# agimus-project/agimus_controller

Hardware: AMD Instinct MI355X
Metric: MPC steps/sec (horizon=100, Panda 7-DoF) (higher is better)
Workload: dtype f64; 1 GPU; Panda 7-DoF sine_wave_configuration_space, ocp_goal_reaching.yaml costs, horizon=100, dt=0.01, batch=1024 independent MPC instances per GPU (seed 1234+b), closed loop on own prediction; horizon=100, batch_per_gpu=1024, global_batch=1024, max_iter=10

## Files before the change

agimus_controller_amd/backend.py:

```python

from __future__ import annotations

import ctypes as C
import os
import pathlib
import subprocess

import numpy as np

from . import _abi

_CSRC = pathlib.Path(__file__).resolve().parent / "csrc"
LIB_PATH = pathlib.Path(os.environ.get("AGX_LIB", _CSRC / "libagimus_hip.so"))
_LIB = None

EXPORTED_SYMBOLS = [
    "agx_last_error", "agx_device_count", "agx_row_nref", "agx_row_nr", "agx_ref_stride",
    "agx_model_create", "agx_model_destroy", "agx_ocp_create", "agx_ocp_destroy", "agx_ocp_set_stream",
    "agx_ocp_sync", "agx_ocp_set_refs", "agx_ocp_set_refs_device", "agx_ocp_solve", "agx_ocp_upload_x0",
    "agx_ocp_upload_warmstart", "agx_ocp_solve_resident", "agx_ocp_download", "agx_ocp_download_first", "agx_ocp_first_packed", "agx_ocp_set_geom_placement", "agx_ocp_reset_duals", "agx_traj_generic_create", "agx_traj_set_horizon_indexes", "agx_ocp_feedback_rollout", "agx_ocp_download_x0", "agx_model_frame_jacobian",
    "agx_ocp_shift_warmstart", "agx_ocp_x0_from_prediction", "agx_ocp_integrate", "agx_model_rnea",
    "agx_model_frame_placement", "agx_ocp_get_residuals", "agx_ocp_calc_diff", "agx_ocp_direction",
    "agx_ocp_time_kernel", "agx_ocp_profile", "agx_traj_sine_create", "agx_traj_set_window",
    "agx_traj_get_point", "agx_traj_warmstart_from_reference", "agx_ocp_mpc_step", "agx_ocp_qp_tiles", "agx_ocp_set_quorum",
    "agx_traj_cartesian_sine_create", "agx_ocp_set_refs_async", "agx_ocp_refs_activate", "agx_ocp_refs_wait", "agx_host_alloc", "agx_host_free",
    "agx_ocp_download_async", "agx_ocp_download_wait",
]


def _run(cmd, verbose):
    res = subprocess.run(cmd, capture_output=True, text=True)
    if verbose or res.returncode != 0:
        print(res.stdout, res.stderr)
    if res.returncode != 0:
        raise RuntimeError(f"{cmd[0]} failed ({res.returncode}): {res.stderr[-2000:]}")


def build(force: bool = False, verbose: bool = False) -> pathlib.Path:
    hdr = _CSRC.parent.parent / "include" / "agimus_hip.h"
    srcs = [_CSRC / "agimus_hip.hip"] + sorted(_CSRC.glob("*.hpp")) + [hdr, _CSRC / "agx_front.py"]
    if not force and LIB_PATH.exists() and LIB_PATH.stat().st_mtime >= max(s.stat().st_mtime for s in srcs):
        return LIB_PATH
    hipcc = os.environ.get("HIPCC", "/opt/rocm/bin/hipcc")
    base = [hipcc, "--offload-arch=gfx950", "-O3", "-std=c++17", "-fPIC"]
    if os.environ.get("AGX_BUILD_SPLIT", "1") == "0":
        _run(base + ["-shared", "-o", str(LIB_PATH), str(srcs[0])], verbose)
        return LIB_PATH
    import importlib.util

    spec = importlib.util.spec_from_file_location("agx_front", _CSRC / "agx_front.py")
    front = importlib.util.module_from_spec(spec)
    spec.loader.exec_module(front)
    obj = _CSRC.parent.parent / "build" / "obj"
    obj.mkdir(parents=True, exist_ok=True)
    names = [n for _, n, _ in front.prototypes(hdr.read_text())]
    procs = []
    for g in front.GROUPS:
        cmd = base + ["-c", f"-I{hdr.parent}"] + front.rename_flags(names, g) + ["-o", str(obj / f"agx_g{g}.o"), str(srcs[0])]
        procs.append((cmd, subprocess.Popen(cmd, stdout=subprocess.PIPE, stderr=subprocess.PIPE, text=True)))
    (obj / "agx_front.cpp").write_text(front.front_source(hdr.read_text()))
    _run(["g++", "-O2", "-std=c++17", "-fPIC", f"-I{hdr.parent}", "-c", "-o", str(obj / "agx_front.o"), str(obj / "agx_front.cpp")], verbose)
    failed = None
    for cmd, p in procs:
        out, err = p.communicate()
        if verbose or p.returncode != 0:
            print(out, err)
        if p.returncode != 0 and failed is None:
            failed = RuntimeError(f"hipcc failed ({p.returncode}) for {cmd[-1]} [{cmd[-3]}]: {err[-2000:]}")
    if failed:
        raise failed
    _run([hipcc, "--offload-arch=gfx950", "-shared", "-fPIC", "-o", str(LIB_PATH)] + [str(obj / f"agx_g{g}.o") for g in front.GROUPS]
         + [str(obj / "agx_front.o")], verbose)
    return LIB_PATH


def lib():
    global _LIB
    if _LIB is None:
        if not LIB_PATH.exists():
# ... 154 lines not shown
        _chk(lib().agx_ocp_upload_x0(self._h, _p(_f8(x0, (self.B, self.nx)))))

    def upload_warmstart(self, xs, us):
        xs = _f8(xs, (self.B, self.T + 1, self.nx))
        us = _f8(us, (self.B, self.T, self.nu))
        _chk(lib().agx_ocp_upload_warmstart(self._h, _p(xs), _p(us)))

    def solve_resident(self, max_iter, max_time=0.0):
        _chk(lib().agx_ocp_solve_resident(self._h, int(max_iter), C.c_double(max_time)))

    def download(self, want_K=True):
        xs = np.empty((self.B, self.T + 1, self.nx))
        us = np.empty((self.B, self.T, self.nu))
        K = np.empty((self.B, self.T, self.nu, self.nx)) if want_K else None
        st = np.zeros(self.B, dtype=_abi.STATUS_DTYPE)
        _chk(lib().agx_ocp_download(self._h, _p(xs), _p(us), _p(K), _p(st)))
        return xs, us, K, st

    def download_first(self, want_status=True, copy=True):
        ptr = C.POINTER(C.c_double)()
        stride = C.c_int(0)
        _chk(lib().agx_ocp_first_packed(self._h, C.byref(ptr), C.byref(stride)))
        addr = C.addressof(ptr.contents)
        cached = getattr(self, "_first_view", None)
        if cached is None or cached[0] != addr:
            cached = (addr, np.ctypeslib.as_array(ptr, shape=(self.B, stride.value)))
            self._first_view = cached
        buf = cached[1]
        nu, nx = self.nu, self.nx
        nk = nu * nx
        us0 = buf[:, :nu]
        K0 = buf[:, nu:nu + nk].reshape(self.B, nu, nx)
        x1 = buf[:, nu + nk:nu + nk + nx]
        if copy:
            us0, K0, x1 = us0.copy(), K0.copy(), x1.copy()
        st = None
        if want_status:
            q = buf[:, nu + nk + nx:]
            names = ("kkt", "cost", "merit", "gap_norm", "iter", "qp_iters", "solved", "flags")
            if copy:
                st = np.zeros(self.B, dtype=_abi.STATUS_DTYPE)
                for k, name in enumerate(names):
                    st[name] = q[:, k] if k < 4 else q[:, k].astype(np.int32)
            else:
                st = {name: q[:, k] for k, name in enumerate(names)}
        return us0, K0, x1, st

    def set_geom_placement(self, frame: int, se3_12):
        _chk(lib().agx_ocp_set_geom_placement(self._h, int(frame), _p(_f8(se3_12).reshape(12))))

    def set_quorum(self, sqp_fraction: float = 1.0, qp_fraction: float = 1.0):
        _chk(lib().agx_ocp_set_quorum(self._h, C.c_double(sqp_fraction), C.c_double(qp_fraction)))

    def reset_duals(self):
        _chk(lib().agx_ocp_reset_duals(self._h))

    def shift_warmstart(self):
        _chk(lib().agx_ocp_shift_warmstart(self._h))

    def x0_from_prediction(self):
        _chk(lib().agx_ocp_x0_from_prediction(self._h))

    def integrate(self, x, u):
        x = _f8(x).reshape(-1, self.nx)
        u = _f8(u).reshape(-1, self.nu)
        out = np.empty_like(x)
        _chk(lib().agx_ocp_integrate(self._h, x.shape[0], _p(x), _p(u), _p(out)))
        return out

    def rnea(self, q, v, a):
        q = _f8(q).reshape(-1, self.nv)
        v = _f8(v).reshape(-1, self.nv)
        a = _f8(a).reshape(-1, self.nv)
        tau = np.empty_like(q)
        _chk(lib().agx_model_rnea(self._h, q.shape[0], _p(q), _p(v), _p(a), _p(tau)))
        return tau

    def frame_placement(self, frame: int, q):
        q = _f8(q).reshape(-1, self.nv)
        out = np.empty((q.shape[0], 12))
        _chk(lib().agx_model_frame_placement(self._h, q.shape[0], int(frame), _p(q), _p(out)))
        return out

    def frame_jacobian(self, frame: int, q, local: bool = False):
        q = _f8(q).reshape(-1, self.nv)
        J = np.empty((q.shape[0], 6, self.nv))
        _chk(lib().agx_model_frame_jacobian(self._h, q.shape[0], int(frame), 1 if local else 0, _p(q), _p(J)))
        return J

    def residuals(self, row: int):
        nr = _abi.row_nr(self.po.running[row].kind, self.nv)
        out = np.empty((self.B, self.T, nr))
        _chk(lib().agx_ocp_get_residuals(self._h, int(row), _p(out)))
        return out

    def calc_diff(self, want_tiles=True):
        tiles = np.empty((self.B, self.T + 1, self.tile)) if want_tiles else None
        _chk(lib().agx_ocp_calc_diff(self._h, _p(tiles)))
        return tiles

    def qp_tiles(self):
        qs, as_ = C.c_int(0), C.c_int(0)
        _chk(lib().agx_ocp_qp_tiles(self._h, None, None, C.byref(qs), C.byref(as_)))
        qt = np.empty((self.B, self.T + 1, qs.value))
        aux = np.empty((self.B, self.T + 1, as_.value))
        _chk(lib().agx_ocp_qp_tiles(self._h, _p(qt), _p(aux), C.byref(qs), C.byref(as_)))
# ... 87 lines not shown
```

agimus_controller_amd/csrc/agimus_hip.hip:

```cpp

#include <hip/hip_runtime.h>

#include <algorithm>
#include <chrono>
#include <cmath>
#include <cstddef>
#include <cstdio>
#include <cstdlib>
#include <cstring>
#include <string>
#include <vector>

#include "agx_kernels.hpp"

namespace {

thread_local std::string g_err;
int fail(const std::string &msg) {
  g_err = msg;
  return -1;
}
#define HIPCHK(expr)                                                                                      \
  do {                                                                                                    \
    hipError_t e_ = (expr);                                                                               \
// ... 33 lines not shown
  int *d_shift_nodes = nullptr;
  bool general = false;
  double *d_auxg = nullptr;
  double *d_qt2 = nullptr, *d_cg = nullptr, *d_cjac = nullptr, *d_y = nullptr, *d_z = nullptr, *d_cx = nullptr, *d_admmstat = nullptr,
         *d_fac = nullptr,
         *d_segP = nullptr;
  bool admm_segments = true;
  int qt_size = 0, aux_size = 0;
  bool k1_lanes = true;
  bool lanes_ok = true;
  bool lanes_coll = false;
  bool speculate = true;
  bool gains_mfma = true;
  bool riccati_mx = true;
  int mx2_S = 0;
  double *d_mx2_elem = nullptr, *d_mx2_bnd = nullptr, *d_mx2_cl = nullptr;
  bool k1_fused = true;
  bool tile_carry = true;
  bool carry_static = false;
  bool carry_armed = false;
  int carry_k0 = 0;
  int head = 0;
  int n_carriable = -1;
  bool frames_uniform = true;
  double quorum_sqp = 1.0, quorum_qp = 1.0;
  bool con_lanes = true;
  bool con_wide = false;
  int con_cs = AGX_MAX_NC;
  bool admm_loop_always = false;
  bool admm_loop = true;
  int n_unfinished = 1 << 30;
  bool fold_publish = false;
  int n_cu = 256;
  bool no_empty = false;
  double *d_ref = nullptr;
  double *d_ref_back = nullptr;
  int *d_frames_back = nullptr;
  bool refs_pending = false, refs_pending_frames = false;
  hipStream_t copy_stream = nullptr;
  hipEvent_t ev_refs = nullptr, ev_snap = nullptr, ev_dl = nullptr;
  double *d_snap = nullptr;
  bool dl_pending = false;
  int *d_frames = nullptr;
  bool frames_set = false;
  DevState *d_state = nullptr;
  int *d_ndone = nullptr;
  unsigned long long *h_ndone = nullptr;
  unsigned long long *h_ndone_dev = nullptr;
  unsigned long long seq = 0;
  unsigned ls_handed = 0, ls_stale = 0;
  bool poll = true;
  double *d_first = nullptr, *h_first = nullptr;
  int first_stride = 0;
  double *d_scratch = nullptr;
  size_t scratch_bytes = 0;
  RefView rv{};
  double *d_traj = nullptr, *d_pts = nullptr;
  double *d_sine = nullptr;
  int n_points = 0;
  std::vector<int> hidx;
  int *d_hidx = nullptr;
  int win_k0 = 0;
  hipEvent_t ev0 = nullptr, ev1 = nullptr, ev_done = nullptr;
  int last_max_iter = 0;
  bool prof = false;
  std::vector<hipEvent_t> prof_ev;
  std::vector<int> prof_kind;
  double prof_ms[3] = {0, 0, 0};
  long long prof_n[3] = {0, 0, 0};
};

namespace {

int set_device(agx_ocp *o) {
  HIPCHK(hipSetDevice(o->device));
  return 0;
}

int pad_capacity(int nv);

void pad_rows(double *dst, const double *src, size_t rows, int blocks, int nvu, int nv, double fill) {
  for (size_t r = 0; r < rows; ++r)
    for (int b = 0; b < blocks; ++b) {
      double *d = dst + (r * blocks + b) * nv;
      const double *q = src + (r * blocks + b) * nvu;
      for (int i = 0; i < nvu; ++i) d[i] = q[i];
      for (int i = nvu; i < nv; ++i) d[i] = fill;
    }
}
void unpad_rows(double *dst, const double *src, size_t rows, int blocks, int nvu, int nv) {
  for (size_t r = 0; r < rows; ++r)
    for (int b = 0; b < blocks; ++b) {
      double *d = dst + (r * blocks + b) * nvu;
      const double *q = src + (r * blocks + b) * nv;
      for (int i = 0; i < nvu; ++i) d[i] = q[i];
    }
}
int up(agx_ocp *o, double *d_dst, const double *h_src, size_t rows, int blocks, double fill = 0.0) {
  if (!o->padded) {
    HIPCHK(hipMemcpyAsync(d_dst, h_src, sizeof(double) * rows * blocks * o->nv, hipMemcpyHostToDevice, o->stream));
    return 0;
  }
  o->stage.resize(rows * blocks * o->nv);
  pad_rows(o->stage.data(), h_src, rows, blocks, o->nvu, o->nv, fill);
  HIPCHK(hipMemcpyAsync(d_dst, o->stage.data(), sizeof(double) * o->stage.size(), hipMemcpyHostToDevice, o->stream));
  HIPCHK(hipStreamSynchronize(o->stream));
  return 0;
}
int down(agx_ocp *o, double *h_dst, const double *d_src, size_t rows, int blocks) {
  if (!o->padded) {
    HIPCHK(hipMemcpyAsync(h_dst, d_src, sizeof(double) * rows * blocks * o->nv, hipMemcpyDeviceToHost, o->stream));
    return 0;
  }
  o->stage.resize(rows * blocks * o->nv);
  HIPCHK(hipMemcpyAsync(o->stage.data(), d_src, sizeof(double) * o->stage.size(), hipMemcpyDeviceToHost, o->stream));
  HIPCHK(hipStreamSynchronize(o->stream));
  unpad_rows(h_dst, o->stage.data(), rows, blocks, o->nvu, o->nv);
  return 0;
}
int down_gains(agx_ocp *o, double *h_dst, const double *d_src, size_t n) {
  if (!o->padded) {
    HIPCHK(hipMemcpyAsync(h_dst, d_src, sizeof(double) * n * o->nu * o->nx, hipMemcpyDeviceToHost, o->stream));
    return 0;
  }
  const int nv = o->nv, nvu = o->nvu;
  o->stage.resize(n * nv * 2 * nv);
  HIPCHK(hipMemcpyAsync(o->stage.data(), d_src, sizeof(double) * o->stage.size(), hipMemcpyDeviceToHost, o->stream));
// ... 618 lines not shown
            if (n_conv < o->B && iter < max_qp) {
              hipLaunchKernelGGL(agx::k_admm_cap, dim3((o->B + 255) / 256), dim3(256), 0, o->stream, o->d_state, o->B, iter);
              HIPCHK(hipGetLastError());
            }
            break;
          }
        }
      }
      const long long units = (long long)o->B * o->T * 64;
      hipLaunchKernelGGL((agx::k_gains_to_u_big<NV>), dim3((int)((units + 255) / 256)), dim3(256), 0, o->stream, o->d_ocp, o->d_aux, o->d_Kws,
                         o->d_Kout, (const DevState *)nullptr);
      HIPCHK(hipGetLastError());
      return 0;
    } else {
      if constexpr (CH) if (o->con_wide) return admm_direction_nv7<NV, CH, true>(o, prefactor);
      return admm_direction_nv7<NV, CH, false>(o, prefactor);
    }
  });
}

int carry_invalidate(agx_ocp *o) {
  o->carry_armed = false;
  if (o->head != 0) {
    o->head = 0;
    HIPCHK(hipMemsetAsync((char *)o->d_ocp + offsetof(DevOcp, head), 0, sizeof(int), o->stream));
  }
  return 0;
}

int adopt_pending_refs(agx_ocp *o) {
  if (!o->refs_pending) return 0;
  if (carry_invalidate(o)) return -1;
  if (o->refs_pending_frames) o->frames_uniform = false;
  HIPCHK(hipStreamWaitEvent(o->stream, o->ev_refs, 0));
  std::swap(o->d_ref, o->d_ref_back);
  if (o->refs_pending_frames) std::swap(o->d_frames, o->d_frames_back);
  o->rv.base = o->d_ref;
  o->rv.bstride = (long long)(o->T + 1) * o->stride;
  o->rv.tstride = o->stride;
  o->rv.term_off = 0;
  o->rv.frames = o->refs_pending_frames ? o->d_frames : nullptr;
  o->refs_pending = false;
  return 0;
}
int ensure_copy_stream(agx_ocp *o) {
  if (o->copy_stream) return 0;
  HIPCHK(hipStreamCreateWithFlags(&o->copy_stream, hipStreamNonBlocking));
  HIPCHK(hipEventCreateWithFlags(&o->ev_refs, hipEventDisableTiming));
  HIPCHK(hipEventCreateWithFlags(&o->ev_snap, hipEventDisableTiming));
  HIPCHK(hipEventCreateWithFlags(&o->ev_dl, hipEventDisableTiming));
  return 0;
}

int line_search_rounds(agx_ocp *o, int it, int max_iter, bool *need_k1, int *n_done_out) {
  double *xs_t = o->d_xs + (size_t)o->B * (o->T + 1) * o->nx, *us_t = o->d_us + (size_t)o->B * o->T * o->nu;
  for (int round = 0; round < 10; ++round) {
    if (o->prof && round == 0 && it == 0) {
      if (prof_mark(o, 0, true)) return -1;
      if (launch_calc_qp(o, true, false, 1)) return -1;
      if (prof_mark(o, 0, false)) return -1;
      if (launch_calc_qp(o, false, true, 1)) return -1;
    } else if (launch_calc_qp(o, false, false, 1)) return -1;
    const unsigned long long seq = ++o->seq;
    int rc = dispatch(o->nv, o->chain, [&](auto NVc, auto CHc) -> int {
      constexpr int NV = decltype(NVc)::value;
      constexpr bool CH = decltype(CHc)::value;
      (void)CH;
      if constexpr (NV <= 7) if (o->has_con) {
        launch_con_eval<NV, CH>(o, xs_t, us_t, 1);
      }
      if constexpr (NV > 7) if (o->has_con) {
        const long long nodes = (long long)o->B * (o->T + 1);
        hipLaunchKernelGGL((agx::k_con_eval_wg<NV>), dim3((int)nodes), dim3(256), 0, o->stream, o->d_model, o->d_ocp, xs_t, us_t, o->d_cg, o->d_cjac,
                           o->d_nodestat, o->d_state, 1);
      }
      if (prof_mark(o, 2, true)) return -1;
      hipLaunchKernelGGL((agx::k_sqp_accept<NV>), dim3(o->B), dim3(128), 0, o->stream, o->d_ocp, o->d_xs, o->d_us, o->d_dx, o->d_du, xs_t, us_t,
                         o->d_qt, o->d_nodestat, o->d_state, it, max_iter, o->d_ndone, host_words(o, true, seq));
      HIPCHK(hipGetLastError());
      return prof_mark(o, 2, false);
    });
    if (rc) return rc;
    if (o->poll && o->fold_publish) {
      if (wait_stamp(o, 1, seq)) return -1;
    } else if (o->poll) {
      hipLaunchKernelGGL(agx::k_publish3, dim3(1), dim3(1), 0, o->stream, o->d_ndone, o->h_ndone_dev + 0, o->h_ndone_dev + 6, o->h_ndone_dev + 7,
                         o->h_ndone_dev + 8, o->h_ndone_dev + 1, seq);
      HIPCHK(hipGetLastError());
      if (wait_stamp(o, 1, seq)) return -1;
    } else {
      o->h_ndone[0] = 0; o->h_ndone[6] = 0; o->h_ndone[7] = 0; o->h_ndone[8] = 0;
      HIPCHK(hipMemcpyAsync(o->h_ndone + 8, o->d_ndone + 6, sizeof(int), hipMemcpyDeviceToHost, o->stream));
      HIPCHK(hipMemcpyAsync(o->h_ndone, o->d_ndone, sizeof(int), hipMemcpyDeviceToHost, o->stream));
      HIPCHK(hipMemcpyAsync(o->h_ndone + 6, o->d_ndone + 3, sizeof(int), hipMemcpyDeviceToHost, o->stream));
      HIPCHK(hipMemcpyAsync(o->h_ndone + 7, o->d_ndone + 4, sizeof(int), hipMemcpyDeviceToHost, o->stream));
      HIPCHK(hipStreamSynchronize(o->stream));
    }
    *n_done_out = (int)__atomic_load_n(o->h_ndone, __ATOMIC_ACQUIRE);
    const unsigned handed = (unsigned)__atomic_load_n(o->h_ndone + 6, __ATOMIC_ACQUIRE);
    const unsigned stale = (unsigned)__atomic_load_n(o->h_ndone + 7, __ATOMIC_ACQUIRE);
    o->n_carriable = (int)__atomic_load_n(o->h_ndone + 8, __ATOMIC_ACQUIRE);
    const bool more = handed != o->ls_handed;
    if (stale != o->ls_stale) *need_k1 = true;
    o->ls_handed = handed;
    o->ls_stale = stale;
    if (!more) break;
  }
  return 0;
}

int solve_resident(agx_ocp *o, int max_iter, double max_time, bool prologue_done = false, int carry_mode = 0) {
  if (max_iter <= 0) max_iter = 1000;
  o->last_max_iter = max_iter;
  o->n_carriable = -1;
  auto t0 = std::chrono::steady_clock::now();
  if (!prologue_done) {
    if (reset_state(o)) return -1;
    hipLaunchKernelGGL(agx::k_pin_x0, dim3((o->B * o->nx + 255) / 256), dim3(256), 0, o->stream, o->d_xs, o->d_x0, o->B, o->T, o->nx);
  }
  bool need_k1 = true;
  bool need_fixup = false;
  int prev_done = 0;
  for (int it = 0; it < max_iter; ++it) {
    const bool pair = o->speculate && it >= 1 && !o->has_con && o->nv <= 7;
    o->n_unfinished = o->B - prev_done;
    if (need_k1) {
      if (it == 0 && carry_mode != 0) {
        if (launch_calc_qp(o, false, false, 0, carry_mode == 2)) return -1;
      } else if (o->prof && it == 0) {
        if (prof_mark(o, 0, true)) return -1;
        if (launch_calc_qp(o, true, false)) return -1;
        if (prof_mark(o, 0, false)) return -1;
        if (launch_calc_qp(o, false, true)) return -1;
      } else if (launch_calc_qp(o, false, false)) return -1;
    }
    need_k1 = false;
    if (prof_mark(o, 1, true)) return -1;
    if (o->has_con && o->admm_prefactor && o->riccati_mx && o->nv <= 7 && !o->general) {
      if (admm_direction(o, true)) return -1;
    } else {
      if (launch_riccati(o, 1, pair, it)) return -1;
      if (o->has_con && admm_direction(o)) return -1;
    }
    if (prof_mark(o, 1, false)) return -1;
    const bool last = it + 1 == max_iter;
    if (prof_mark(o, 2, true)) return -1;
    const unsigned long long seq_head = ++o->seq;
    if (launch_step(o, it, max_iter, 1, !o->has_con, true, seq_head)) return -1;
    if (prof_mark(o, 2, false)) return -1;
    int n_done = 0;
    if (!pair && !o->has_con && (last || max_time > 0.0 || o->quorum_sqp < 1.0)) {
      if (launch_gains(o, 4)) return -1;
    }
    bool searching = true;
    if (o->poll && o->fold_publish && it >= 1) {
      if (wait_stamp(o, 1, seq_head)) return -1;
      n_done = (int)__atomic_load_n(o->h_ndone, __ATOMIC_ACQUIRE);
      o->n_carriable = (int)__atomic_load_n(o->h_ndone + 8, __ATOMIC_ACQUIRE);
      searching = n_done < o->B;
    } else if (o->prof || o->no_empty) {
      if (read_int(o, o->d_ndone, 0, 1, &n_done)) return -1;
      searching = n_done < o->B;
      if (!searching && read_int(o, o->d_ndone + 6, 8, 1, &o->n_carriable)) return -1;
    }
    if (searching && line_search_rounds(o, it, max_iter, &need_k1, &n_done)) return -1;
    if (last) { need_fixup = need_fixup || !pair; break; }
    if (!pair && n_done > prev_done) need_fixup = true;
    prev_done = n_done;
    if (n_done >= quorum_count(o->B, o->quorum_sqp)) {
      if (n_done < o->B) o->last_max_iter = it + 1;
      break;
    }
    if (max_time > 0.0) {
      const double el = std::chrono::duration<double>(std::chrono::steady_clock::now() - t0).count();
      if (el > max_time) { need_fixup = need_fixup || !pair; o->last_max_iter = it + 1; break; }
    }
  }
  if (!o->has_con && need_fixup && launch_gains(o, 2)) return -1;
  return prof_collect(o);
}

}

extern "C" {

const char *agx_last_error(void) { return g_err.c_str(); }

int agx_device_count(void) {
  int n = 0;
  if (hipGetDeviceCount(&n) != hipSuccess) return 0;
  return n;
}

int agx_row_nref(int kind, int nv) {
  switch (kind) {
    case AGX_RES_STATE: return 2 * nv;
    case AGX_RES_CONTROL: return nv;
    case AGX_RES_CONTROL_GRAV: return 0;
    case AGX_RES_FRAME_PLACEMENT: return 12;
    case AGX_RES_FRAME_TRANSLATION: return 3;
    case AGX_RES_FRAME_ROTATION: return 9;
    case AGX_RES_FRAME_VELOCITY: return 6;
    case AGX_RES_COLLISION: return 0;
  }
  return -1;
}
int agx_row_nr(int kind, int nv) {
  switch (kind) {
    case AGX_RES_STATE: return 2 * nv;
    case AGX_RES_CONTROL: return nv;
    case AGX_RES_CONTROL_GRAV: return nv;
    case AGX_RES_FRAME_PLACEMENT: return 6;
    case AGX_RES_FRAME_TRANSLATION: return 3;
    case AGX_RES_FRAME_ROTATION: return 3;
    case AGX_RES_FRAME_VELOCITY: return 6;
    case AGX_RES_COLLISION: return 1;
  }
  return -1;
// ... 60 lines not shown
  return 0;
}
void agx_model_destroy(agx_model *m) { delete m; }

int agx_ocp_create(const agx_model *m, const agx_ocp_desc *d, int batch, int device, agx_ocp **out) {
  if (!m || !d || !out) return fail("agx_ocp_create: null argument");
  if (batch < 1) return fail("agx_ocp_create: batch must be positive");
  if (d->horizon < 1) return fail("agx_ocp_create: horizon must be positive");
  if (d->n_running_rows > AGX_MAX_ROWS || d->n_terminal_rows > AGX_MAX_ROWS) return fail("agx_ocp_create: too many cost rows");
  int ndev = 0;
  if (hipGetDeviceCount(&ndev) != hipSuccess || ndev <= 0) return fail("agx_ocp_create: no HIP device available (this library has no CPU path)");
  if (device < 0 || device >= ndev) return fail("agx_ocp_create: bad device index");
  for (int r = 0; r < d->n_running_rows + d->n_terminal_rows; ++r) {
    const agx_cost_row &row = r < d->n_running_rows ? d->running_rows[r] : d->terminal_rows[r - d->n_running_rows];
    switch (row.kind) {
      case AGX_RES_STATE: case AGX_RES_CONTROL: case AGX_RES_FRAME_PLACEMENT: case AGX_RES_FRAME_TRANSLATION: case AGX_RES_FRAME_ROTATION:
      case AGX_RES_COLLISION: break;
      case AGX_RES_CONTROL_GRAV: case AGX_RES_FRAME_VELOCITY:
        if (m->h.nv > 7) return fail("agx_ocp_create: ControlGrav / FrameVelocity rows are implemented for nv <= 7");
        if (row.kind == AGX_RES_FRAME_VELOCITY && (row.frame < 0 || row.frame >= m->h.nframes || row.frame_b < 0 || row.frame_b > 2))
          return fail("agx_ocp_create: FrameVelocity row needs a valid frame and a reference frame 0 (WORLD), 1 (LOCAL) or 2 (LOCAL_WORLD_ALIGNED)");
        break;
      default: return fail("agx_ocp_create: residual kind " + std::to_string(row.kind) + " is not implemented on the HIP path yet");
    }
    if (row.activation != AGX_ACT_WEIGHTED_QUAD && (row.kind == AGX_RES_CONTROL_GRAV || row.kind == AGX_RES_FRAME_VELOCITY))
      return fail("agx_ocp_create: ActivationModelExp / QuadExp are not implemented for ControlGrav / FrameVelocity residuals");
    if (row.activation != AGX_ACT_WEIGHTED_QUAD && !(row.alpha > 0.0)) return fail("agx_ocp_create: activation alpha must be positive");
    if ((row.kind == AGX_RES_FRAME_PLACEMENT || row.kind == AGX_RES_FRAME_TRANSLATION || row.kind == AGX_RES_FRAME_ROTATION) &&
        (row.frame < 0 || row.frame >= m->h.nframes))
      return fail("agx_ocp_create: frame id out of range");
    if (row.kind == AGX_RES_COLLISION) {
      if (row.frame < 0 || row.frame >= m->h.nframes || row.frame_b < 0 || row.frame_b >= m->h.nframes)
        return fail("agx_ocp_create: collision pair refers to a geometry frame out of range");
      if (!agx::frame_has_geometry(m->h, row.frame) || !agx::frame_has_geometry(m->h, row.frame_b))
        return fail("agx_ocp_create: collision pair refers to a frame without geometry (radius 0, no box)");
      if (agx::frame_is_box(m->h, row.frame) && agx::frame_is_box(m->h, row.frame_b))
        return fail("agx_ocp_create: box / box collision pairs are not supported");
    }
  }
  agx_ocp *o = new agx_ocp();
  o->hm = m->h;
  o->nv = m->h.nv; o->nx = 2 * o->nv; o->nu = o->nv;
  o->chain = m->h.is_chain != 0;
  if (const char *e = getenv("AGX_K1_LANES")) o->k1_lanes = (e[0] != '0');
  if (const char *e = getenv("AGX_SPECULATE_GAINS")) o->speculate = (e[0] != '0');
  if (const char *e = getenv("AGX_GAINS_MFMA")) o->gains_mfma = (e[0] != '0');
  if (const char *e = getenv("AGX_RICCATI_MX")) o->riccati_mx = (e[0] != '0');
  if (const char *e = getenv("AGX_NO_EMPTY_LAUNCHES")) o->no_empty = (e[0] != '0');
  o->fold_publish = batch <= 204;
  if (const char *e = getenv("AGX_FOLD_PUBLISH")) o->fold_publish = (e[0] != '0');
  if (const char *e = getenv("AGX_ADMM_LOOP")) { o->admm_loop = (e[0] != '0'); o->admm_loop_always = (e[0] == '2'); }
  if (const char *e = getenv("AGX_K1_FUSED")) o->k1_fused = (e[0] != '0');
  if (const char *e = getenv("AGX_TILE_CARRY")) o->tile_carry = (e[0] != '0');
  o->T = d->horizon; o->B = batch; o->device = device;
  {
    int n = 0;
    if (hipDeviceGetAttribute(&n, hipDeviceAttributeMultiprocessorCount, device) == hipSuccess && n > 0) o->n_cu = n;
  }
  o->tile = AGX_TILE_DOUBLES(o->nv);
  const int ld = o->nv <= 8 ? 8 : 32;
  o->qt_size = 6 * o->nv * ld + 5 * ld + 8;
  o->aux_size = 4 * o->nv * ld + 3 * ld;
  o->stride = agx_ref_stride(d, o->nv);
  o->dt.assign(d->dt, d->dt + d->horizon);
  std::memset(&o->ho, 0, sizeof(o->ho));
  o->ho.T = o->T; o->ho.B = o->B; o->ho.stride = o->stride;
  fill_rows(d->running_rows, d->n_running_rows, o->nv, m->nvu, o->ho.rows[0]);
  fill_rows(d->terminal_rows, d->n_terminal_rows, o->nv, m->nvu, o->ho.rows[1]);
  o->ho.tol = d->termination_tolerance;
  o->ho.mu_dyn = d->mu_dynamic;
  o->ho.mu_con = d->mu_constraint;
  o->nvu = m->nvu;
  o->padded = o->nvu != o->nv;
  o->stride_u = agx_ref_stride(d, o->nvu);
  if (o->padded) {
    for (int lay = 0; lay < 2; ++lay) {
      const DevRows &R = o->ho.rows[lay];
      o->refmap[lay].assign(o->stride, -1);
      o->reffill[lay].assign(o->stride, 0.0);
      int off_u = 0;
      for (int r = 0; r < R.n; ++r) {
        const int kind = R.kind[r], nref_u = agx_row_nref(kind, o->nvu), nr_u = agx_row_nr(kind, o->nvu);
        o->refmap[lay][R.off[r]] = off_u;
        for (int k = 0; k < R.nref[r]; ++k) {
          const int ku = user_component(kind, k, o->nv, o->nvu, true);
          o->refmap[lay][R.off[r] + 1 + k] = ku >= 0 ? off_u + 1 + ku : -1;
        }
        for (int k = 0; k < R.nr[r]; ++k) {
          const int ku = user_component(kind, k, o->nv, o->nvu, false);
          o->refmap[lay][R.off[r] + 1 + R.nref[r] + k] = ku >= 0 ? off_u + 1 + nref_u + ku : -1;
          if (ku < 0) o->reffill[lay][R.off[r] + 1 + R.nref[r] + k] = 1.0;
        }
        off_u += 1 + nref_u + nr_u;
      }
    }
  }
  {
    const int wc_r = wide_class(d->running_constraints, d->n_running_constraints, false),
              wc_t = wide_class(d->terminal_constraints, d->n_terminal_constraints, true);
    const bool wide_model = o->nv <= 7 && o->chain, wide_ok = wide_model && wc_r == 0 && wc_t == 0;
    bool wide = false;
    if (const char *e = getenv("AGX_CON_WIDE")) wide = wide_ok && e[0] == '1';
    if (!wide && (fill_cons(d->running_constraints, d->n_running_constraints, o->nv, o->nvu, m->h, o->ho.cons[0], false) ||
                  fill_cons(d->terminal_constraints, d->n_terminal_constraints, o->nv, o->nvu, m->h, o->ho.cons[1], true))) {
      if (wide_model && (wc_r == 2 || wc_t == 2)) {
        delete o;
// ... 156 lines not shown
  (void)hipEventCreate(&o->ev1);
  (void)hipEventCreateWithFlags(&o->ev_done, hipEventDisableTiming);
  o->rv.base = o->d_ref;
  o->rv.bstride = (long long)(T + 1) * o->stride;
  o->rv.tstride = o->stride;
  o->rv.term_off = 0;
  o->rv.frames = nullptr;
  if (reset_state(o) || hipStreamSynchronize(o->stream) != hipSuccess) { agx_ocp_destroy(o); return fail("agx_ocp_create: state reset failed"); }
  *out = o;
  return 0;
}

void agx_ocp_destroy(agx_ocp *o) {
  if (!o) return;
  (void)hipSetDevice(o->device);
  if (o->stream) (void)hipStreamSynchronize(o->stream);
  if (o->copy_stream) (void)hipStreamSynchronize(o->copy_stream);
  void *ptrs[] = {o->d_mx2_elem, o->d_mx2_bnd, o->d_mx2_cl, o->d_ref_back, o->d_frames_back, o->d_snap, o->d_model, o->d_ocp, o->d_dt, o->d_xs, o->d_us, o->d_x0, o->d_tiles, o->d_Kws, o->d_kws, o->d_Kout, o->d_dx,
                  o->d_du, o->d_ref, o->d_frames, o->d_state, o->d_ndone, o->d_scratch, o->d_traj, o->d_pts, o->d_sine, o->d_qt, o->d_aux, o->d_w, o->d_nodestat,
                  o->d_qt2, o->d_cg, o->d_cjac, o->d_y, o->d_z, o->d_cx, o->d_admmstat, o->d_fac, o->d_hidx, o->d_auxg, o->d_shift_nodes, o->d_segP, o->d_Kws_lqr, o->d_kws_lqr};
  for (void *p : ptrs)
    if (p) (void)hipFree(p);
  if (o->h_ndone) (void)hipHostFree(o->h_ndone);
  if (o->ev0) (void)hipEventDestroy(o->ev0);
  if (o->ev1) (void)hipEventDestroy(o->ev1);
  if (o->ev_done) (void)hipEventDestroy(o->ev_done);
  if (o->ev_refs) (void)hipEventDestroy(o->ev_refs);
  if (o->ev_snap) (void)hipEventDestroy(o->ev_snap);
  if (o->ev_dl) (void)hipEventDestroy(o->ev_dl);
  if (o->copy_stream) (void)hipStreamDestroy(o->copy_stream);
  if (o->d_first && !o->poll) (void)hipFree(o->d_first);
  if (o->h_first) (void)hipHostFree(o->h_first);
  if (o->own_stream && o->stream) (void)hipStreamDestroy(o->stream);
  delete o;
}

int agx_ocp_set_stream(agx_ocp *o, void *hip_stream) {
  if (!o) return fail("null handle");
  if (set_device(o)) return -1;
  if (o->stream) HIPCHK(hipStreamSynchronize(o->stream));
  if (hip_stream) {
    if (o->own_stream && o->stream) (void)hipStreamDestroy(o->stream);
    o->stream = (hipStream_t)hip_stream;
    o->own_stream = false;
  } else if (!o->own_stream) {
    HIPCHK(hipStreamCreateWithFlags(&o->stream, hipStreamNonBlocking));
    o->own_stream = true;
  }
  return 0;
}

int agx_ocp_sync(agx_ocp *o) {
  if (!o) return fail("null handle");
  if (set_device(o)) return -1;
  HIPCHK(hipStreamSynchronize(o->stream));
  return 0;
}

int agx_ocp_set_quorum(agx_ocp *o, double sqp_fraction, double qp_fraction) {
  if (!o) return fail("null handle");
  if (!(sqp_fraction > 0.0 && sqp_fraction <= 1.0) || !(qp_fraction > 0.0 && qp_fraction <= 1.0))
    return fail("agx_ocp_set_quorum: fractions must be in (0, 1]");
  o->quorum_sqp = sqp_fraction;
  o->quorum_qp = qp_fraction;
  return 0;
}

int agx_ocp_reset_duals(agx_ocp *o) {
  if (!o) return fail("null handle");
  if (set_device(o)) return -1;
  if (o->has_con) HIPCHK(hipMemsetAsync(o->d_y, 0, sizeof(double) * (size_t)o->B * (o->T + 1) * o->con_cs, o->stream));
  hipLaunchKernelGGL(agx::k_reset_rho, dim3((o->B + 255) / 256), dim3(256), 0, o->stream, o->d_state, o->B);
  HIPCHK(hipGetLastError());
  HIPCHK(hipStreamSynchronize(o->stream));
  return 0;
}

int agx_ocp_set_geom_placement(agx_ocp *o, int frame, const double *se3) {
  if (!o || !se3) return fail("agx_ocp_set_geom_placement: null argument");
  if (frame < 0 || frame >= o->hm.nframes) return fail("agx_ocp_set_geom_placement: frame out of range");
  if (set_device(o)) return -1;
  if (carry_invalidate(o)) return -1;
  std::memcpy(o->hm.frame_placement[frame], se3, sizeof(double) * 12);
  HIPCHK(hipMemcpyAsync((char *)o->d_model + offsetof(DevModel, frame_placement) + sizeof(double) * 12 * frame, o->hm.frame_placement[frame],
                        sizeof(double) * 12, hipMemcpyHostToDevice, o->stream));
  HIPCHK(hipStreamSynchronize(o->stream));
  return 0;
}

int agx_ocp_set_refs(agx_ocp *o, const double *ref_tile, const int32_t *frame_ids) {
  if (!o || !ref_tile) return fail("agx_ocp_set_refs: null argument");
  if (set_device(o)) return -1;
  if (carry_invalidate(o)) return -1;
  if (frame_ids) o->frames_uniform = false;
  if (o->refs_pending) { HIPCHK(hipEventSynchronize(o->ev_refs)); o->refs_pending = false; }
  const size_t n = (size_t)o->B * (o->T + 1);
  if (o->padded) {
    o->stage.resize(n * o->stride);
    pad_ref_tile(o, o->stage.data(), ref_tile, o->B, o->T);
    ref_tile = o->stage.data();
  }
  HIPCHK(hipMemcpyAsync(o->d_ref, ref_tile, sizeof(double) * n * o->stride, hipMemcpyHostToDevice, o->stream));
  if (frame_ids) HIPCHK(hipMemcpyAsync(o->d_frames, frame_ids, sizeof(int) * n * AGX_MAX_ROWS, hipMemcpyHostToDevice, o->stream));
  HIPCHK(hipStreamSynchronize(o->stream));
  o->rv.base = o->d_ref;
  o->rv.bstride = (long long)(o->T + 1) * o->stride;
  o->rv.tstride = o->stride;
  o->rv.term_off = 0;
// ... 115 lines not shown
  return 0;
}

int agx_ocp_upload_x0(agx_ocp *o, const double *x0) {
  if (!o || !x0) return fail("agx_ocp_upload_x0: null argument");
  if (set_device(o)) return -1;
  if (up(o, o->d_x0, x0, o->B, 2)) return -1;
  HIPCHK(hipStreamSynchronize(o->stream));
  return 0;
}

int agx_ocp_upload_warmstart(agx_ocp *o, const double *xs_ws, const double *us_ws) {
  if (!o || !xs_ws || !us_ws) return fail("agx_ocp_upload_warmstart: null argument");
  if (set_device(o)) return -1;
  if (carry_invalidate(o)) return -1;
  if (up(o, o->d_xs, xs_ws, (size_t)o->B * (o->T + 1), 2)) return -1;
  if (up(o, o->d_us, us_ws, (size_t)o->B * o->T, 1)) return -1;
  HIPCHK(hipStreamSynchronize(o->stream));
  return 0;
}

int agx_ocp_solve_resident(agx_ocp *o, int max_iter, double max_time) {
  if (!o) return fail("null handle");
  if (set_device(o)) return -1;
  if (carry_invalidate(o)) return -1;
  return solve_resident(o, max_iter, max_time);
}

int agx_ocp_download(agx_ocp *o, double *xs, double *us, double *K, agx_status *st) {
  if (!o) return fail("null handle");
  if (set_device(o)) return -1;
  const size_t B = o->B, T = o->T, nx = o->nx, nu = o->nu;
  (void)nx; (void)nu;
  if (xs && down(o, xs, o->d_xs, B * (T + 1), 2)) return -1;
  if (us && down(o, us, o->d_us, B * T, 1)) return -1;
  if (K && down_gains(o, K, o->d_Kout, B * T)) return -1;
  std::vector<DevState> hs;
  if (st) {
    hs.resize(B);
    HIPCHK(hipMemcpyAsync(hs.data(), o->d_state, sizeof(DevState) * B, hipMemcpyDeviceToHost, o->stream));
  }
  HIPCHK(hipStreamSynchronize(o->stream));
  if (st)
    for (size_t b = 0; b < B; ++b) {
      st[b].kkt = hs[b].kkt; st[b].cost = hs[b].cost; st[b].merit = hs[b].merit; st[b].gap_norm = hs[b].gap;
      st[b].iter = hs[b].done ? hs[b].iter : o->last_max_iter;
      st[b].qp_iters = hs[b].qp_iters; st[b].solved = hs[b].solved; st[b].flags = hs[b].flags;
    }
  return 0;
}

int agx_ocp_first_packed(agx_ocp *o, const double **host, int *stride) {
  if (!o || !host) return fail("agx_ocp_first_packed: null argument");
  if (set_device(o)) return -1;
  const int FS = o->nu + o->nu * o->nx + o->nx + 8;
  if (!o->h_first) {
    if (o->poll && hipHostMalloc((void **)&o->h_first, sizeof(double) * (size_t)o->B * FS, hipHostMallocMapped | hipHostMallocCoherent) != hipSuccess) {
      (void)hipGetLastError();
      o->poll = false;
    }
    if (!o->poll) HIPCHK(hipHostMalloc((void **)&o->h_first, sizeof(double) * (size_t)o->B * FS, hipHostMallocDefault));
    if (o->poll) {
      HIPCHK(hipHostGetDevicePointer((void **)&o->d_first, o->h_first, 0));
    } else {
      HIPCHK(hipMalloc((void **)&o->d_first, sizeof(double) * (size_t)o->B * FS));
    }
    o->first_stride = FS;
  }
  const long long n = (long long)o->B * FS;
  hipLaunchKernelGGL(agx::k_pack_first, dim3((int)((n + 255) / 256)), dim3(256), 0, o->stream, o->d_us, o->d_Kout, o->d_xs, o->d_state,
                     o->d_first, o->B, o->T, o->nx, o->nu, o->last_max_iter);
  HIPCHK(hipGetLastError());
  if (o->poll) {
    const unsigned long long seq = ++o->seq;
    if (publish(o, 3, 2, o->d_ndone, seq)) return -1;
    if (wait_stamp(o, 2, seq)) return -1;
  } else {
    HIPCHK(hipMemcpyAsync(o->h_first, o->d_first, sizeof(double) * n, hipMemcpyDeviceToHost, o->stream));
    HIPCHK(hipStreamSynchronize(o->stream));
  }
  if (o->padded) {
    const int nv = o->nv, nvu = o->nvu, FSu = nvu + nvu * 2 * nvu + 2 * nvu + 8;
    o->h_first_u.resize((size_t)o->B * FSu);
    for (int b = 0; b < o->B; ++b) {
      const double *r = o->h_first + (size_t)b * FS;
      double *w = o->h_first_u.data() + (size_t)b * FSu;
      unpad_rows(w, r, 1, 1, nvu, nv);
      for (int i = 0; i < nvu; ++i) unpad_rows(w + nvu + (size_t)i * 2 * nvu, r + nv + (size_t)i * 2 * nv, 1, 2, nvu, nv);
      unpad_rows(w + nvu + nvu * 2 * nvu, r + nv + nv * 2 * nv, 1, 2, nvu, nv);
      std::memcpy(w + nvu + nvu * 2 * nvu + 2 * nvu, r + nv + nv * 2 * nv + 2 * nv, sizeof(double) * 8);
    }
    *host = o->h_first_u.data();
    if (stride) *stride = FSu;
    return 0;
  }
  *host = o->h_first;
  if (stride) *stride = FS;
  return 0;
}

int agx_ocp_download_first(agx_ocp *o, double *us0, double *K0, double *x1, agx_status *st) {
  const double *h = nullptr;
  int FS = 0;
  if (agx_ocp_first_packed(o, &h, &FS)) return -1;
  const int nu = o->nvu, nx = 2 * o->nvu, nk = nu * nx;
  for (int b = 0; b < o->B; ++b) {
    const double *r = h + (size_t)b * FS;
    if (us0) std::memcpy(us0 + (size_t)b * nu, r, sizeof(double) * nu);
    if (K0) std::memcpy(K0 + (size_t)b * nk, r + nu, sizeof(double) * nk);
    if (x1) std::memcpy(x1 + (size_t)b * nx, r + nu + nk, sizeof(double) * nx);
    if (st) {
      const double *q = r + nu + nk + nx;
      st[b].kkt = q[0]; st[b].cost = q[1]; st[b].merit = q[2]; st[b].gap_norm = q[3];
      st[b].iter = (int)q[4]; st[b].qp_iters = (int)q[5]; st[b].solved = (int)q[6]; st[b].flags = (int)q[7];
    }
  }
  return 0;
}

int agx_ocp_solve(agx_ocp *o, const double *x0, const double *xs_ws, const double *us_ws, int max_iter, double max_time,
                  double *xs, double *us, double *K, agx_status *st) {
  if (!o || !x0 || !xs_ws || !us_ws) return fail("agx_ocp_solve: null argument");
  if (agx_ocp_upload_x0(o, x0)) return -1;
  if (agx_ocp_upload_warmstart(o, xs_ws, us_ws)) return -1;
  if (solve_resident(o, max_iter, max_time)) return -1;
  return agx_ocp_download(o, xs, us, K, st);
}

int agx_ocp_shift_warmstart(agx_ocp *o) {
  if (!o) return fail("null handle");
// ... 525 lines not shown
  if (n_substeps < 1 || !(dt_sub > 0.0)) return fail("agx_ocp_feedback_rollout: bad sub-stepping");
  if (set_device(o)) return -1;
  double *d_dist = nullptr;
  if (disturbance) {
    if (ensure_scratch(o, sizeof(double) * o->B * o->nu)) return -1;
    d_dist = o->d_scratch;
    if (up(o, d_dist, disturbance, o->B, 1)) return -1;
  }
  return dispatch(o->nv, o->chain, [&](auto NVc, auto CHc) -> int {
    constexpr int NV = decltype(NVc)::value;
    constexpr bool CH = decltype(CHc)::value;
    hipLaunchKernelGGL((agx::k_feedback_rollout<NV, CH>), dim3((o->B + 63) / 64), dim3(64), 0, o->stream, o->d_model, o->d_us, o->d_Kout, o->d_x0,
                       d_dist, o->B, o->T, n_substeps, dt_sub);
    HIPCHK(hipGetLastError());
    if (disturbance) HIPCHK(hipStreamSynchronize(o->stream));
    return 0;
  });
}

int agx_ocp_mpc_step(agx_ocp *o, int k0, int max_iter, int first) {
  if (!o) return fail("null handle");
  if (set_device(o)) return -1;
  if (agx_traj_set_window(o, k0)) return -1;
  bool prologue_done = false;
  const size_t lds = sizeof(double) * (size_t)o->T * (o->nx + o->nu);
  const bool one_launch = o->nv <= 8 && lds <= 60 * 1024;
  const bool carry = o->carry_static && o->carry_armed && first != 1 && k0 == o->carry_k0 + 1 && one_launch && o->hidx.empty() && o->frames_uniform;
  const int carry_mode = !carry ? 0 : (o->n_carriable == o->B ? 2 : 1);
  if (!carry && carry_invalidate(o)) return -1;
  o->carry_armed = false;
  if (first == 1) {
    if (ws_from_ref(o, k0, 1)) return -1;
  } else {
    if (one_launch) {
      if (carry) o->head = (o->head + 1) % o->T;
      int rc = dispatch(o->nv, o->chain, [&](auto NVc, auto CHc) -> int {
        constexpr int NV = decltype(NVc)::value;
        constexpr bool CH = decltype(CHc)::value;
        if constexpr (NV <= 8) {
          hipLaunchKernelGGL((agx::k_mpc_prologue<NV, CH>), dim3(o->B), dim3(128), lds, o->stream, o->d_model, o->d_ocp, o->d_dt, o->d_xs,
                             o->d_us, o->d_x0, o->d_state, o->d_ndone, first == 0 ? 1 : 0, carry ? 1 : 0, o->head,
                             (int *)((char *)o->d_ocp + offsetof(DevOcp, head)));
          HIPCHK(hipGetLastError());
        }
        return 0;
      });
      if (rc) return rc;
      prologue_done = true;
    } else {
      if (first == 0 && agx_ocp_x0_from_prediction(o)) return -1;
      if (agx_ocp_shift_warmstart(o)) return -1;
    }
  }
  if (solve_resident(o, max_iter, 0.0, prologue_done, carry_mode)) return -1;
  o->carry_armed = o->carry_static;
  o->carry_k0 = k0;
  return 0;
}

}
```

include/agimus_hip.h:

```cpp
#ifndef AGIMUS_HIP_H
#define AGIMUS_HIP_H

#include <stddef.h>
#include <stdint.h>

#ifdef __cplusplus
extern "C" {
#endif

#define AGX_MAX_ROWS 8
#define AGX_MAX_NV 32

enum agx_residual_kind {
  AGX_RES_STATE = 0,
  AGX_RES_CONTROL = 1,
  AGX_RES_CONTROL_GRAV = 2,
  AGX_RES_FRAME_PLACEMENT = 3,
  AGX_RES_FRAME_TRANSLATION = 4,
  AGX_RES_FRAME_ROTATION = 5,
  AGX_RES_FRAME_VELOCITY = 6,
  AGX_RES_COLLISION = 7
};

enum agx_activation_kind {
// ... 42 lines not shown
  const double *frame_box;
} agx_model_desc;

typedef struct agx_ocp_desc {
  int32_t horizon;
  const double *dt;
  int32_t n_running_rows;
  const agx_cost_row *running_rows;
  int32_t n_terminal_rows;
  const agx_cost_row *terminal_rows;
  double termination_tolerance;
  int32_t max_qp_iters;
  double eps_abs, eps_rel;
  double mu_dynamic, mu_constraint;
  int32_t use_filter_line_search;
  int32_t n_running_constraints;
  const agx_constraint_row *running_constraints;
  int32_t n_terminal_constraints;
  const agx_constraint_row *terminal_constraints;
} agx_ocp_desc;

typedef struct agx_status {
  double kkt;
  double cost;
  double merit;
  double gap_norm;
  int32_t iter;
  int32_t qp_iters;
  int32_t solved;
  int32_t flags;
} agx_status;

#define AGX_TILE_DOUBLES(nv) (4 * (nv) * (nv) + 2 * (nv) * (nv) + 2 * (nv) + 2 * (nv) + (nv) + 4 * (nv) * (nv) + 2 * (nv) * (nv) + (nv) * (nv) + 1)

typedef struct agx_model agx_model;
typedef struct agx_ocp agx_ocp;

const char *agx_last_error(void);
int agx_device_count(void);

int agx_row_nref(int kind, int nv);
int agx_row_nr(int kind, int nv);
int agx_ref_stride(const agx_ocp_desc *desc, int nv);

int agx_model_create(const agx_model_desc *desc, agx_model **out);
void agx_model_destroy(agx_model *m);

int agx_ocp_create(const agx_model *m, const agx_ocp_desc *desc, int batch, int device, agx_ocp **out);
void agx_ocp_destroy(agx_ocp *ocp);
int agx_ocp_set_stream(agx_ocp *ocp, void *hip_stream);
int agx_ocp_sync(agx_ocp *ocp);
int agx_ocp_set_geom_placement(agx_ocp *ocp, int frame, const double *se3);
int agx_ocp_set_quorum(agx_ocp *ocp, double sqp_fraction, double qp_fraction);
int agx_ocp_reset_duals(agx_ocp *ocp);

int agx_ocp_set_refs(agx_ocp *ocp, const double *ref_tile, const int32_t *frame_ids);
int agx_ocp_set_refs_async(agx_ocp *ocp, const double *ref_tile, const int32_t *frame_ids);
int agx_ocp_refs_activate(agx_ocp *ocp);
int agx_ocp_refs_wait(agx_ocp *ocp);
int agx_host_alloc(size_t bytes, void **out);
int agx_host_free(void *p);
int agx_ocp_set_refs_device(agx_ocp *ocp, const double *d_ref_tile, const int32_t *d_frame_ids, int adopt);

int agx_ocp_solve(agx_ocp *ocp, const double *x0, const double *xs_ws, const double *us_ws,
                  int max_iter, double max_time, double *xs, double *us, double *K, agx_status *st);

int agx_ocp_upload_x0(agx_ocp *ocp, const double *x0);
int agx_ocp_upload_warmstart(agx_ocp *ocp, const double *xs_ws, const double *us_ws);
int agx_ocp_solve_resident(agx_ocp *ocp, int max_iter, double max_time);
int agx_ocp_download(agx_ocp *ocp, double *xs, double *us, double *K, agx_status *st);
int agx_ocp_download_async(agx_ocp *ocp, double *xs, double *us, double *K);
int agx_ocp_download_wait(agx_ocp *ocp);
int agx_ocp_download_first(agx_ocp *ocp, double *us0, double *K0, double *x1, agx_status *st);
int agx_ocp_first_packed(agx_ocp *ocp, const double **host, int *stride);

int agx_ocp_shift_warmstart(agx_ocp *ocp);
int agx_ocp_x0_from_prediction(agx_ocp *ocp);

int agx_ocp_integrate(agx_ocp *ocp, int n, const double *x, const double *u, double *xnext);

int agx_model_rnea(agx_ocp *ocp, int n, const double *q, const double *v, const double *a, double *tau);
int agx_model_frame_placement(agx_ocp *ocp, int n, int frame, const double *q, double *out);
int agx_model_frame_jacobian(agx_ocp *ocp, int n, int frame, int local, const double *q, double *J);

int agx_ocp_get_residuals(agx_ocp *ocp, int row, double *out);

int agx_ocp_calc_diff(agx_ocp *ocp, double *tiles);
int agx_ocp_direction(agx_ocp *ocp, double *K, double *k, double *dx, double *du, double *kkt);
int agx_ocp_qp_tiles(agx_ocp *ocp, double *qt, double *aux, int *qt_size, int *aux_size);
int agx_ocp_time_kernel(agx_ocp *ocp, int which, int reps, double *avg_ms);

int agx_ocp_profile(agx_ocp *ocp, int enable, double *ms_sum, long long *count);

int agx_traj_sine_create(agx_ocp *ocp, int n_points, double dt, const double *q0, const double *amp,
                         const double *pulsation, const double *scale_duration, const double *t0,
                         const double *w_q, const double *w_qdot, const double *w_effort,
                         const double *w_pose, int frame);
int agx_traj_generic_create(agx_ocp *ocp, int n_points, const double *q, const double *dq, const double *ddq,
                            const double *w_q, const double *w_qdot, const double *w_effort, const double *w_pose, int frame);
int agx_traj_cartesian_sine_create(agx_ocp *ocp, int n_points, double dt, const double *q0, const double *amp,
                                   const double *pulsation, double scale_duration, double precision, int it_max,
                                   const double *w_q, const double *w_qdot, const double *w_effort, const double *w_pose,
                                   int frame);
int agx_traj_set_window(agx_ocp *ocp, int k0);
int agx_traj_set_horizon_indexes(agx_ocp *ocp, const int32_t *idx);
int agx_traj_get_point(agx_ocp *ocp, int k, double *q, double *v, double *a, double *u, double *pose);
// ... 11 lines not shown
```

Baseline: 1.196 million MPC steps/s.

## Queue first-step pack speculatively and predict solver convergence iteration to skip host round-trips

At the end of an MPC step the pack of first-step outputs is queued on the stream right away, so agx_ocp_first_packed can just wait for the stamp instead of launching and publishing itself. The solver also remembers the iteration where all instances finished last step. On that iteration it publishes done-counts and queues the pack speculatively, which avoids a separate line-search round-trip. This aims to cut host-device synchronisation latency per step, at the cost of extra state tracking and a possibly wasted pack when the prediction is wrong.

```diff
diff --git a/agimus_controller_amd/backend.py b/agimus_controller_amd/backend.py
--- a/agimus_controller_amd/backend.py
+++ b/agimus_controller_amd/backend.py
@@ -24,7 +24,7 @@
     "agx_ocp_time_kernel", "agx_ocp_profile", "agx_traj_sine_create", "agx_traj_set_window",
     "agx_traj_get_point", "agx_traj_warmstart_from_reference", "agx_ocp_mpc_step", "agx_ocp_qp_tiles", "agx_ocp_set_quorum",
     "agx_traj_cartesian_sine_create", "agx_ocp_set_refs_async", "agx_ocp_refs_activate", "agx_ocp_refs_wait", "agx_host_alloc", "agx_host_free",
-    "agx_ocp_download_async", "agx_ocp_download_wait",
+    "agx_ocp_download_async", "agx_ocp_download_wait", "agx_ocp_host_loop_counts",
 ]
 
 
@@ -285,6 +285,11 @@
     def set_quorum(self, sqp_fraction: float = 1.0, qp_fraction: float = 1.0):
         _chk(lib().agx_ocp_set_quorum(self._h, C.c_double(sqp_fraction), C.c_double(qp_fraction)))
 
+    def host_loop_counts(self):
+        a, b = C.c_int(0), C.c_int(0)
+        _chk(lib().agx_ocp_host_loop_counts(self._h, C.byref(a), C.byref(b)))
+        return a.value, b.value
+
     def reset_duals(self):
         _chk(lib().agx_ocp_reset_duals(self._h))
 
diff --git a/agimus_controller_amd/csrc/agimus_hip.hip b/agimus_controller_amd/csrc/agimus_hip.hip
--- a/agimus_controller_amd/csrc/agimus_hip.hip
+++ b/agimus_controller_amd/csrc/agimus_hip.hip
@@ -109,6 +109,13 @@
   bool poll = true;
   double *d_first = nullptr, *h_first = nullptr;
   int first_stride = 0;
+  bool queue_ahead = true;
+  bool in_mpc = false;
+  int head_end_it = -1;
+  bool first_fresh = false;
+  unsigned long long first_seq = 0;
+  unsigned long long spec_pack_seq = 0;
+  int heads_asked = 0, spec_packs_used = 0;
   double *d_scratch = nullptr;
   size_t scratch_bytes = 0;
   RefView rv{};
@@ -129,7 +136,8 @@
 
 namespace {
 
-int set_device(agx_ocp *o) {
+int set_device(agx_ocp *o, bool keeps_results = false) {
+  if (!keeps_results) o->first_fresh = false;
   HIPCHK(hipSetDevice(o->device));
   return 0;
 }
@@ -854,6 +862,15 @@
   return 0;
 }
 
+int queue_pack_first(agx_ocp *o, unsigned long long *seq_out) {
+  const long long n = (long long)o->B * o->first_stride;
+  hipLaunchKernelGGL(agx::k_pack_first, dim3((int)((n + 255) / 256)), dim3(256), 0, o->stream, o->d_us, o->d_Kout, o->d_xs, o->d_state,
+                     o->d_first, o->B, o->T, o->nx, o->nu, o->last_max_iter);
+  HIPCHK(hipGetLastError());
+  *seq_out = ++o->seq;
+  return publish(o, 3, 2, o->d_ndone, *seq_out);
+}
+
 int line_search_rounds(agx_ocp *o, int it, int max_iter, bool *need_k1, int *n_done_out) {
   double *xs_t = o->d_xs + (size_t)o->B * (o->T + 1) * o->nx, *us_t = o->d_us + (size_t)o->B * o->T * o->nu;
   for (int round = 0; round < 10; ++round) {
@@ -923,6 +940,11 @@
   bool need_k1 = true;
   bool need_fixup = false;
   int prev_done = 0;
+  const bool ask_head = o->queue_ahead && o->in_mpc && o->poll && !o->fold_publish && !o->has_con && !o->general && o->nv <= 7 && !o->prof &&
+                        !o->no_empty;
+  const int pred_head_it = o->head_end_it;
+  o->head_end_it = -1;
+  o->spec_pack_seq = 0;
   for (int it = 0; it < max_iter; ++it) {
     const bool pair = o->speculate && it >= 1 && !o->has_con && o->nv <= 7;
     o->n_unfinished = o->B - prev_done;
@@ -964,8 +986,27 @@
       if (read_int(o, o->d_ndone, 0, 1, &n_done)) return -1;
       searching = n_done < o->B;
       if (!searching && read_int(o, o->d_ndone + 6, 8, 1, &o->n_carriable)) return -1;
-    }
-    if (searching && line_search_rounds(o, it, max_iter, &need_k1, &n_done)) return -1;
+    } else if (ask_head && it >= 1 && pred_head_it == it) {
+      const unsigned long long seq = ++o->seq;
+      ++o->heads_asked;
+      hipLaunchKernelGGL(agx::k_publish3, dim3(1), dim3(1), 0, o->stream, o->d_ndone, o->h_ndone_dev + 0, o->h_ndone_dev + 6, o->h_ndone_dev + 7,
+                         o->h_ndone_dev + 8, o->h_ndone_dev + 1, seq);
+      HIPCHK(hipGetLastError());
+      unsigned long long pack_seq = 0;
+      if (o->h_first && pair && !need_fixup && queue_pack_first(o, &pack_seq)) return -1;
+      if (wait_stamp(o, 1, seq)) return -1;
+      n_done = (int)__atomic_load_n(o->h_ndone, __ATOMIC_ACQUIRE);
+      o->n_carriable = (int)__atomic_load_n(o->h_ndone + 8, __ATOMIC_ACQUIRE);
+      searching = n_done < o->B;
+      if (!searching) o->spec_pack_seq = pack_seq;
+    }
+    if (!searching && o->in_mpc) o->head_end_it = it;
+    if (searching) {
+      const unsigned handed0 = o->ls_handed, stale0 = o->ls_stale;
+      if (line_search_rounds(o, it, max_iter, &need_k1, &n_done)) return -1;
+      if (o->in_mpc && ask_head && it >= 1 && pred_head_it != it && n_done >= o->B && handed0 == o->ls_handed && stale0 == o->ls_stale)
+        o->head_end_it = it;
+    }
     if (last) { need_fixup = need_fixup || !pair; break; }
     if (!pair && n_done > prev_done) need_fixup = true;
     prev_done = n_done;
@@ -1132,6 +1173,7 @@
   if (const char *e = getenv("AGX_ADMM_LOOP")) { o->admm_loop = (e[0] != '0'); o->admm_loop_always = (e[0] == '2'); }
   if (const char *e = getenv("AGX_K1_FUSED")) o->k1_fused = (e[0] != '0');
   if (const char *e = getenv("AGX_TILE_CARRY")) o->tile_carry = (e[0] != '0');
+  if (const char *e = getenv("AGX_QUEUE_AHEAD")) o->queue_ahead = (e[0] != '0');
   o->T = d->horizon; o->B = batch; o->device = device;
   {
     int n = 0;
@@ -1394,8 +1436,15 @@
 
 int agx_ocp_sync(agx_ocp *o) {
   if (!o) return fail("null handle");
-  if (set_device(o)) return -1;
-  HIPCHK(hipStreamSynchronize(o->stream));
+  if (set_device(o, true)) return -1;
+  HIPCHK(hipStreamSynchronize(o->stream));
+  return 0;
+}
+
+int agx_ocp_host_loop_counts(agx_ocp *o, int *heads_asked, int *spec_packs_used) {
+  if (!o || !heads_asked || !spec_packs_used) return fail("agx_ocp_host_loop_counts: null argument");
+  *heads_asked = o->heads_asked;
+  *spec_packs_used = o->spec_packs_used;
   return 0;
 }
 
@@ -1617,6 +1666,7 @@
 
 int agx_ocp_first_packed(agx_ocp *o, const double **host, int *stride) {
   if (!o || !host) return fail("agx_ocp_first_packed: null argument");
+  const bool fresh = o->first_fresh && o->poll && o->h_first;
   if (set_device(o)) return -1;
   const int FS = o->nu + o->nu * o->nx + o->nx + 8;
   if (!o->h_first) {
@@ -1633,14 +1683,17 @@
     o->first_stride = FS;
   }
   const long long n = (long long)o->B * FS;
-  hipLaunchKernelGGL(agx::k_pack_first, dim3((int)((n + 255) / 256)), dim3(256), 0, o->stream, o->d_us, o->d_Kout, o->d_xs, o->d_state,
-                     o->d_first, o->B, o->T, o->nx, o->nu, o->last_max_iter);
-  HIPCHK(hipGetLastError());
-  if (o->poll) {
-    const unsigned long long seq = ++o->seq;
-    if (publish(o, 3, 2, o->d_ndone, seq)) return -1;
+  if (fresh) {
+    if (wait_stamp(o, 2, o->first_seq)) return -1;
+    o->first_fresh = true;
+  } else if (o->poll) {
+    unsigned long long seq = 0;
+    if (queue_pack_first(o, &seq)) return -1;
     if (wait_stamp(o, 2, seq)) return -1;
   } else {
+    hipLaunchKernelGGL(agx::k_pack_first, dim3((int)((n + 255) / 256)), dim3(256), 0, o->stream, o->d_us, o->d_Kout, o->d_xs, o->d_state,
+                       o->d_first, o->B, o->T, o->nx, o->nu, o->last_max_iter);
+    HIPCHK(hipGetLastError());
     HIPCHK(hipMemcpyAsync(o->h_first, o->d_first, sizeof(double) * n, hipMemcpyDeviceToHost, o->stream));
     HIPCHK(hipStreamSynchronize(o->stream));
   }
@@ -2272,10 +2325,20 @@
       if (agx_ocp_shift_warmstart(o)) return -1;
     }
   }
-  if (solve_resident(o, max_iter, 0.0, prologue_done, carry_mode)) return -1;
+  o->in_mpc = true;
+  const int rc_solve = solve_resident(o, max_iter, 0.0, prologue_done, carry_mode);
+  o->in_mpc = false;
+  if (rc_solve) { o->head_end_it = -1; return -1; }
   o->carry_armed = o->carry_static;
   o->carry_k0 = k0;
-  return 0;
-}
-
-}
+  if (o->queue_ahead && o->poll && o->h_first && !o->has_con && !o->general && o->nv <= 7 && !o->prof && !o->no_empty) {
+    unsigned long long seq = o->spec_pack_seq;
+    if (seq) ++o->spec_packs_used;
+    else if (queue_pack_first(o, &seq)) return -1;
+    o->first_seq = seq;
+    o->first_fresh = true;
+  }
+  return 0;
+}
+
+}
diff --git a/include/agimus_hip.h b/include/agimus_hip.h
--- a/include/agimus_hip.h
+++ b/include/agimus_hip.h
@@ -118,6 +118,7 @@
 int agx_ocp_sync(agx_ocp *ocp);
 int agx_ocp_set_geom_placement(agx_ocp *ocp, int frame, const double *se3);
 int agx_ocp_set_quorum(agx_ocp *ocp, double sqp_fraction, double qp_fraction);
+int agx_ocp_host_loop_counts(agx_ocp *ocp, int *heads_asked, int *spec_packs_used);
 int agx_ocp_reset_duals(agx_ocp *ocp);
 
 int agx_ocp_set_refs(agx_ocp *ocp, const double *ref_tile, const int32_t *frame_ids);
```

Measured after the change: 1.226 million MPC steps/s, median of 6. 2.5% higher.
